# williamleif/GraphSAGE

Hardware: NVIDIA H100
Metric: seed_nodes_per_sec (higher is better)
Workload: dtype f32

## Files before the change

### graphsage_b200/_lib.py

```python
import ctypes
import os

import torch

_HERE = os.path.dirname(os.path.abspath(__file__))
LIB_PATH = os.path.join(_HERE, "csrc", "libgraphsage_b200.so")

ABI_VERSION = 2
GS_F32, GS_BF16, GS_F64 = 0, 1, 2
ACT_NONE, ACT_RELU = 0, 1
COMBINE_ADD, COMBINE_CONCAT = 0, 1
MATH_FP32_SIMT, MATH_TF32X3, MATH_TF32, MATH_BF16 = 0, 1, 2, 3
CSR_MEAN, CSR_MEAN_SELF, CSR_MAX = 0, 1, 2
MAX_SEGMENTS = 4

c_i32, c_i64, c_u64, c_vp = ctypes.c_int32, ctypes.c_int64, ctypes.c_uint64, ctypes.c_void_p


class Segment(ctypes.Structure):
    _fields_ = [("self_ids", c_vp), ("neigh_ids", c_vp), ("self_row0", c_i64), ("neigh_row0", c_i64),
                ("n", c_i64), ("k", c_i32), ("_pad", c_i32), ("out_row0", c_i64)]


MAX_SHARDS = 16


class ShardedTable(ctypes.Structure):
    _fields_ = [("base", c_vp * MAX_SHARDS), ("row_start", c_i64 * (MAX_SHARDS + 1)), ("n_shards", c_i32),
                ("my_shard", c_i32), ("n_global_rows", c_i64), ("zero_row", c_i64), ("remap", c_vp)]


class GemmPart(ctypes.Structure):
    _fields_ = [("A", c_vp), ("lda", c_i64), ("K", c_i32), ("B", c_vp), ("ldb", c_i64), ("N", c_i32)]


MAX_EMBED_LISTS = 8
MAX_UNIQUE_SAMPLED = 1024
UNIQUE_DRAW_BUDGET = 1 << 20
WALK_MAX_WALKS = 1 << 20
WALK_MAX_LEN = 33


class EmbedGradList(ctypes.Structure):
    _fields_ = [("ids", c_vp), ("grad", c_vp), ("ldg", c_i64), ("n", c_i64), ("group", c_i32), ("scale", ctypes.c_float)]


class DropoutSite(ctypes.Structure):
    _fields_ = [("seed", c_u64), ("call", ctypes.c_uint32), ("rate", ctypes.c_float), ("call_dev", c_vp)]
# ... 28 lines not shown
    "gs_ipc_import": (c_i32, [ctypes.c_char_p, ctypes.POINTER(c_vp)]),
    "gs_ipc_close": (c_i32, [c_vp]),
    "gs_gather_rows_f32": (c_i32, [c_vp, c_i32, c_i64, c_i32, c_i64, c_vp, c_i64, c_i64, c_vp, c_i64, c_vp]),
    "gs_cast_rows_bf16": (c_i32, [c_vp, c_i64, c_i32, c_i64, c_vp, c_i64, c_vp]),
    "gs_rmat_degrees": (c_i32, [c_i32, c_i64, ctypes.c_double, ctypes.c_double, ctypes.c_double, ctypes.c_double,
                                ctypes.c_double, c_u64, c_u64, c_u64, c_u64, c_vp, c_vp]),
    "gs_rmat_fill": (c_i32, [c_i32, c_i64, ctypes.c_double, ctypes.c_double, ctypes.c_double, ctypes.c_double, c_u64, c_u64,
                             c_u64, c_u64, c_vp, c_vp, c_vp, c_i64, c_i64, c_vp]),
    "gs_segment_max": (c_i32, [c_vp, c_i64, c_i32, c_i32, c_i64, c_vp, c_i64, c_vp]),
    "gs_sage_gemm_workspace_bytes": (c_i64, [c_i64, ctypes.POINTER(GemmPart), c_i32, c_i32]),
    "gs_sage_gemm": (c_i32, [c_i64, ctypes.POINTER(GemmPart), c_i32, c_i32, c_vp, c_i32, c_i32, c_vp, c_i64, c_vp,
                             c_vp]),
    "gs_sage_gemm_pack": (c_i32, [ctypes.POINTER(GemmPart), c_i32, c_i32, c_vp, c_vp]),
    "gs_sage_gemm_prepacked": (c_i32, [c_i64, ctypes.POINTER(GemmPart), c_i32, c_i32, c_vp, c_i32, c_i32, c_vp, c_i64,
                                       c_vp, c_vp]),
    "gs_gather_mean_img_bytes": (c_i64, [c_i64, c_i32, c_i32]),
    "gs_gather_mean_img": (c_i32, [c_vp, c_i64, ctypes.POINTER(ShardedTable), c_i32, c_vp, c_i32, c_i64, ctypes.POINTER(Segment),
                                   c_i32, c_i32, c_i32, c_vp, c_vp]),
    "gs_sage_gemm_img": (c_i32, [c_i64, ctypes.POINTER(GemmPart), c_i32, c_i32, c_vp, c_i32, c_vp, c_i64, c_vp, c_vp, c_i32,
                                 c_vp]),
    "gs_sage_layer_small": (c_i32, [c_vp, c_i64, c_i32, c_i64, ctypes.POINTER(Segment), c_i32, ctypes.POINTER(GemmPart),
                                    c_i32, c_i32, c_vp, c_i32, c_i32, c_vp, c_i64, c_vp, c_u64, c_vp]),
    "gs_maxpool_mlp_workspace_bytes": (c_i64, [c_i32, c_i32]),
    "gs_maxpool_mlp_pack": (c_i32, [c_vp, c_i64, c_i32, c_i32, c_vp, c_vp]),
    "gs_maxpool_mlp_fused": (c_i32, [c_vp, c_i64, c_i32, c_i64, c_vp, c_i64, c_i64, c_i32, c_vp, c_vp, c_i32, c_vp, c_i64,
                                     c_vp]),
    "gs_meanpool_mlp_fused": (c_i32, [c_vp, c_i64, c_i32, c_i64, c_vp, c_i64, c_i64, c_i32, c_vp, c_vp, c_i32, c_vp, c_i64,
                                      c_vp]),
    "gs_pool_mlp_dp_bytes": (c_i64, [c_i64, c_i32, c_i32]),
    "gs_pool_mlp_backward_dp": (c_i32, [c_vp, c_i64, c_i32, c_i64, c_vp, c_i64, c_i64, c_i32, c_vp, c_vp, c_i32, c_vp, c_i64,
# ... 94 lines not shown
```

### graphsage_b200/aggregators.py

```python
import torch

from . import ops
from .inits import glorot, zeros
from .layers import Dense, Layer, act_code, identity, relu

_DEFAULT_MATH = [ops.MATH_FP32_SIMT]
_MATH_NAMES = {"fp32": ops.MATH_FP32_SIMT, "simt": ops.MATH_FP32_SIMT, "tf32x3": ops.MATH_TF32X3,
               "tf32": ops.MATH_TF32, "bf16": ops.MATH_BF16}


def set_default_math(mode):
    _DEFAULT_MATH[0] = _MATH_NAMES[mode] if isinstance(mode, str) else int(mode)


def _dropout(x, p):
    return torch.nn.functional.dropout(x, p=float(p), training=True) if p else x


def _dense_segment(n, k):
    return [ops.make_segment(n, k)]


def _rows(src, ids, row0, n, f32=False, out=None):
    if f32:
# ... 104 lines not shown
                             (means, self.neigh_input_dim, self.vars["neigh_weights"])], self._combine())

    def aggregate_rows(self, src, segments, final=None, src_persistent=False):
        if self.dropout:
            raise NotImplementedError("dropout > 0 uses the dense call path")
        y = self._small_layer(src, segments, [(None, self.input_dim, self.vars["self_weights"]),
                                              (None, self.neigh_input_dim, self.vars["neigh_weights"])],
                              self._combine(), False, final)
        if y is not None:
            return y
        y = self._image_layer(src, segments, [(None, self.input_dim, self.vars["self_weights"]),
                                              (None, self.neigh_input_dim, self.vars["neigh_weights"])],
                              self._combine(), False, True)
        if y is not None:
            return y
        xs, xm = ops.gather_mean(src, segments, want_self=True)
        return self._finish([(xs, self.input_dim, self.vars["self_weights"]),
                             (xm, self.neigh_input_dim, self.vars["neigh_weights"])], self._combine())


class GCNAggregator(_SageAggregator):

    def __init__(self, input_dim, output_dim, neigh_input_dim=None, dropout=0., bias=False, act=relu, name=None,
                 concat=False, device="cuda", **kwargs):
        super(GCNAggregator, self).__init__(**kwargs)
        self.dropout = dropout
        self.bias = bias
        self.act = act
        self.concat = concat
        if neigh_input_dim is None:
            neigh_input_dim = input_dim
# ... 222 lines not shown
```

### graphsage_b200/csrc/common.cuh

```cuda
#pragma once
#include <cuda_runtime.h>
#include <math.h>
#include <stdint.h>
#include <stdio.h>
#include <string.h>

#include "../../include/graphsage_b200.h"

namespace gs {

void set_error(const char* fmt, ...);
int32_t cuda_fail(cudaError_t e, const char* what);
int32_t tuning(const char* key, int32_t dflt);
int32_t ensure_dyn_smem(const void* kernel, int bytes);

#define GS_REQUIRE(cond, ...)            \
  do {                                   \
    if (!(cond)) {                       \
      gs::set_error(__VA_ARGS__);        \
      return GS_ERR_INVALID_ARG;         \
    }                                    \
  } while (0)

#define GS_CUDA(expr)                                        \
// ... 143 lines not shown
__device__ __forceinline__ void bulk_wait_read() {
  asm volatile("cp.async.bulk.wait_group.read %0;" ::"n"(N) : "memory");
}
template <int N>
__device__ __forceinline__ void bulk_wait() {
  asm volatile("cp.async.bulk.wait_group %0;" ::"n"(N) : "memory");
}

__device__ __forceinline__ float4 ldg_nc_f4(const float4* p) {
  float4 r;
  asm volatile("ld.global.nc.L1::no_allocate.v4.f32 {%0,%1,%2,%3}, [%4];"
               : "=f"(r.x), "=f"(r.y), "=f"(r.z), "=f"(r.w)
               : "l"(p));
  return r;
}
#endif

}
```

### graphsage_b200/csrc/gather.cu

```cuda
#include "common.cuh"

namespace gs {

struct SegTable {
  gs_segment s[GS_MAX_SEGMENTS];
  int32_t n_segments;
  int64_t total_rows;
};

__device__ __forceinline__ int find_segment(const SegTable& t, int64_t r, int64_t& local) {
  int si = 0;
  int64_t base = 0, end = 0;
#pragma unroll
  for (int q = 0; q < GS_MAX_SEGMENTS - 1; ++q) {
    if (q < t.n_segments - 1) {
      end += t.s[q].n;
      if (r >= end) {
        base = end;
        si = q + 1;
      }
    }
  }
  local = r - base;
  return si;
// ... 221 lines not shown
  const int kb = c >> 3, chunk = c & 7;
  const int64_t mt = orow >> 7;
  const int r = (int)(orow & 127);
  unsigned char* dst = im.base + ((((int64_t)part * im.n_mtiles + mt) * im.kblocks + kb) * 2) * 16384 +
                       (uint32_t)(r * 128 + ((chunk ^ (r & 7)) << 4));
  uint4 hi, lo;
  hi.x = __float_as_uint(v.x) & 0xFFFFE000u; hi.y = __float_as_uint(v.y) & 0xFFFFE000u;
  hi.z = __float_as_uint(v.z) & 0xFFFFE000u; hi.w = __float_as_uint(v.w) & 0xFFFFE000u;
  lo.x = __float_as_uint(v.x - __uint_as_float(hi.x)) & 0xFFFFE000u; lo.y = __float_as_uint(v.y - __uint_as_float(hi.y)) & 0xFFFFE000u;
  lo.z = __float_as_uint(v.z - __uint_as_float(hi.z)) & 0xFFFFE000u; lo.w = __float_as_uint(v.w - __uint_as_float(hi.w)) & 0xFFFFE000u;
  *reinterpret_cast<uint4*>(dst) = hi;
  *reinterpret_cast<uint4*>(dst + 16384) = lo;
}

template <class Rows, bool kDrop>
__global__ void __launch_bounds__(192) gather_mean_tma2_kernel(const __grid_constant__ Rows rows_of, int F,
                                                               const __grid_constant__ SegTable tab,
                                                               int include_self, float* __restrict__ out_self,
                                                               float* __restrict__ out_mean, int64_t out_pitch,
                                                               int row_bytes, const __grid_constant__ GatherImg img,
                                                               const __grid_constant__ DropTab drop) {
  extern __shared__ __align__(128) unsigned char smem[];
  __shared__ __align__(8) uint64_t bar[2];
  __shared__ uint32_t drop_off[2 * GS_MAX_SEGMENTS];
  if (threadIdx.x == 0) {
    mbar_init(&bar[0], 1);
    mbar_init(&bar[1], 1);
    fence_mbar_init();
  }
  if constexpr (kDrop) {
    if (threadIdx.x < 2 * GS_MAX_SEGMENTS) {
      const int s = threadIdx.x % GS_MAX_SEGMENTS;
      drop_off[threadIdx.x] = drop_call_offset(threadIdx.x < GS_MAX_SEGMENTS ? drop.neigh[s] : drop.self[s]);
    }
  }
  __syncthreads();
  const int ncol4 = (int)(out_pitch >> 2);
  const int row_f4 = row_bytes >> 4;
  const size_t buf_bytes = (size_t)kGroupRows * row_bytes;

  int64_t r_issue = blockIdx.x;
  int g_issue = 0;
  auto issue = [&](int buf) -> bool {
    if (r_issue >= tab.total_rows) return false;
    int64_t i;
    const gs_segment& sg = tab.s[find_segment(tab, r_issue, i)];
    const int k = sg.k;
    const int rows_total = k + 1;
    const int first = g_issue * kGroupRows;
    const int cnt = min(kGroupRows, rows_total - first);
    if (threadIdx.x < 32) {
      if (threadIdx.x == 0) mbar_expect_tx(&bar[buf], (uint32_t)(cnt * row_bytes));
      __syncwarp();
      for (int j = threadIdx.x; j < cnt; j += 32) {
        const int jj = first + j;
        int64_t id;
        if (jj < k) id = sg.neigh_ids ? (int64_t)sg.neigh_ids[i * k + jj] : sg.neigh_row0 + i * k + jj;
        else id = sg.self_ids ? (int64_t)sg.self_ids[i] : sg.self_row0 + i;
        bulk_g2s(smem + buf * buf_bytes + (size_t)j * row_bytes, rows_of.row(id), (uint32_t)row_bytes, &bar[buf]);
      }
    }
    if (first + cnt >= rows_total) { r_issue += gridDim.x; g_issue = 0; } else { ++g_issue; }
    return true;
  };

  uint32_t phase[2] = {0u, 0u};
  int buf = 0;
  bool have = issue(0);
  int64_t r = blockIdx.x;
  int g = 0;
  float4 acc[2];
  acc[0] = acc[1] = make_float4(0.f, 0.f, 0.f, 0.f);
  while (have) {
    const bool have_next = issue(buf ^ 1);
    int64_t i;
    const int si = find_segment(tab, r, i);
    const gs_segment& sg = tab.s[si];
    const int k = sg.k;
    const int rows_total = k + 1;
    const int first = g * kGroupRows;
    const int cnt = min(kGroupRows, rows_total - first);
    const bool last = first + cnt >= rows_total;
    mbar_wait(&bar[buf], phase[buf]);
    phase[buf] ^= 1u;
    const float4* rows = reinterpret_cast<const float4*>(smem + buf * buf_bytes);
    const int nn = last ? cnt - 1 : cnt;
    DropSite nsite{};
    if constexpr (kDrop) nsite = with_call_offset(drop.neigh[si], drop_off[si]);
#pragma unroll
    for (int q = 0; q < 2; ++q) {
      const int c = threadIdx.x + q * blockDim.x;
      if (c < ncol4 && c * 4 < F) {
        float4 a = acc[q];
        for (int j = 0; j < nn; ++j) {
          float4 v = rows[j * row_f4 + c];
          if constexpr (kDrop) v = drop4(nsite, i * k + first + j, (uint32_t)c, v);
          a.x += v.x; a.y += v.y; a.z += v.z; a.w += v.w;
        }
        acc[q] = a;
      }
    }
    if (last) {
      const int64_t orow = sg.out_row0 + i;
      const int ncol_img = img.base ? img.kblocks * 8 : 0;
#pragma unroll
      for (int q = 0; q < 2; ++q) {
        const int c = threadIdx.x + q * blockDim.x;
        if (c < ncol4 || c < ncol_img) {
          float4 a = make_float4(0.f, 0.f, 0.f, 0.f), sv = a;
          if (c < ncol4 && c * 4 < F) {
            a = acc[q];
            sv = rows[(cnt - 1) * row_f4 + c];
            if constexpr (kDrop) sv = drop4(with_call_offset(drop.self[si], drop_off[GS_MAX_SEGMENTS + si]), i, (uint32_t)c, sv);
            const float div = (float)(k + (include_self ? 1 : 0));
            if (include_self) { a.x += sv.x; a.y += sv.y; a.z += sv.z; a.w += sv.w; }
            a.x /= div; a.y /= div; a.z /= div; a.w /= div;
            a = mask_tail(a, c * 4, F);
            sv = mask_tail(sv, c * 4, F);
          }
          if (c < ncol4) {
            if (out_mean) reinterpret_cast<float4*>(out_mean + orow * out_pitch)[c] = a;
            if (out_self) reinterpret_cast<float4*>(out_self + orow * out_pitch)[c] = sv;
          }
          if (c < ncol_img) {
            if (img.want_self) gather_img_store(img, 0, orow, c, sv);
            gather_img_store(img, img.want_self ? 1 : 0, orow, c, a);
          }
          if (c < ncol4) acc[q] = make_float4(0.f, 0.f, 0.f, 0.f);
// ... 1011 lines not shown
```

### graphsage_b200/csrc/gemm_api.cu

```cuda
#include "common.cuh"

namespace gs {
int32_t sage_gemm_simt(int64_t M, const gs_gemm_part* parts, int32_t n_parts, int32_t combine, const float* bias,
                       int32_t act, float* out, int64_t ldo, cudaStream_t st);
int64_t sage_gemm_tc_workspace(int64_t M, const gs_gemm_part* parts, int32_t n_parts, int32_t math);
int32_t sage_gemm_tc_img(int64_t M, const gs_gemm_part* parts, int32_t n_parts, int32_t combine, const float* bias, int32_t act,
                         float* out, int64_t ldo, const void* workspace, const void* a_images, int32_t a_part0, cudaStream_t st);
int32_t sage_gemm_tc(int64_t M, const gs_gemm_part* parts, int32_t n_parts, int32_t combine, const float* bias,
                     int32_t act, int32_t math, float* out, int64_t ldo, const void* workspace, cudaStream_t st);
int32_t sage_gemm_tc_pack(const gs_gemm_part* parts, int32_t n_parts, int32_t math, void* workspace, cudaStream_t st);
}

static int32_t check_parts(int64_t M, const gs_gemm_part* parts, int32_t n_parts, int32_t combine, bool need_a = true) {
  GS_REQUIRE(M >= 0, "gs_sage_gemm: M < 0");
  GS_REQUIRE(parts && (n_parts == 1 || n_parts == 2), "gs_sage_gemm: n_parts must be 1 or 2 (got %d)", n_parts);
  GS_REQUIRE(combine == GS_COMBINE_ADD || combine == GS_COMBINE_CONCAT, "gs_sage_gemm: combine=%d", combine);
  for (int i = 0; i < n_parts; ++i) {
    GS_REQUIRE(parts[i].K >= 1 && parts[i].N >= 1, "gs_sage_gemm: part %d has K=%d N=%d", i, parts[i].K, parts[i].N);
    GS_REQUIRE(parts[i].lda >= parts[i].K && parts[i].ldb >= parts[i].N, "gs_sage_gemm: part %d leading dims too small", i);
    GS_REQUIRE(M == 0 || ((parts[i].A || !need_a) && parts[i].B), "gs_sage_gemm: part %d NULL operand", i);
  }
  if (n_parts == 2 && combine == GS_COMBINE_ADD)
    GS_REQUIRE(parts[0].N == parts[1].N, "gs_sage_gemm: ADD needs equal N (%d vs %d)", parts[0].N, parts[1].N);
  return GS_OK;
// ... 5 lines not shown
  if (!parts_host || n_parts < 1 || n_parts > 2 || M < 0) return -1;
  if (math == GS_MATH_FP32_SIMT) return 0;
  return gs::sage_gemm_tc_workspace(M, parts_host, n_parts, math);
}

static bool is_tc(int32_t math) { return math == GS_MATH_TF32X3 || math == GS_MATH_TF32 || math == GS_MATH_BF16; }

int32_t gs_sage_gemm_pack(const gs_gemm_part* parts_host, int32_t n_parts, int32_t math, void* workspace, void* stream) {
  int32_t rc = check_parts(1, parts_host, n_parts, GS_COMBINE_CONCAT, false);
  if (rc != GS_OK) return rc;
  if (math == GS_MATH_FP32_SIMT) return GS_OK;
  GS_REQUIRE(is_tc(math), "gs_sage_gemm_pack: unknown math mode %d", math);
  return gs::sage_gemm_tc_pack(parts_host, n_parts, math, workspace, (cudaStream_t)stream);
}

int32_t gs_sage_gemm_prepacked(int64_t M, const gs_gemm_part* parts_host, int32_t n_parts, int32_t combine,
                               const float* bias, int32_t act, int32_t math, float* out, int64_t ldo,
                               const void* workspace, void* stream) {
  int32_t rc = check_parts(M, parts_host, n_parts, combine);
  if (rc != GS_OK) return rc;
  if (M == 0) return GS_OK;
  GS_REQUIRE(out, "gs_sage_gemm: out is NULL");
  int ntot = parts_host[0].N + ((n_parts == 2 && combine == GS_COMBINE_CONCAT) ? parts_host[1].N : 0);
  GS_REQUIRE(ldo >= ntot, "gs_sage_gemm: ldo=%lld < output width %d", (long long)ldo, ntot);
  GS_REQUIRE(act == GS_ACT_NONE || act == GS_ACT_RELU, "gs_sage_gemm: act=%d", act);
  if (math == GS_MATH_FP32_SIMT)
    return gs::sage_gemm_simt(M, parts_host, n_parts, combine, bias, act, out, ldo, (cudaStream_t)stream);
  GS_REQUIRE(is_tc(math), "gs_sage_gemm: unknown math mode %d", math);
  return gs::sage_gemm_tc(M, parts_host, n_parts, combine, bias, act, math, out, ldo, workspace, (cudaStream_t)stream);
}

int32_t gs_sage_gemm_img(int64_t M, const gs_gemm_part* parts_host, int32_t n_parts, int32_t combine, const float* bias,
                         int32_t act, float* out, int64_t ldo, const void* workspace, const void* a_images,
                         int32_t a_part0, void* stream) {
  GS_REQUIRE(parts_host && n_parts >= 1 && n_parts <= 2, "gs_sage_gemm_img: n_parts must be 1 or 2");
  for (int i = 0; i < n_parts; ++i)
    GS_REQUIRE(parts_host[i].B && parts_host[i].K >= 1 && parts_host[i].N >= 1 && parts_host[i].ldb >= parts_host[i].N,
               "gs_sage_gemm_img: bad part %d", i);
  GS_REQUIRE(combine == GS_COMBINE_CONCAT || n_parts == 1 || parts_host[0].N == parts_host[1].N,
             "gs_sage_gemm_img: ADD needs equal output widths");
  if (M == 0) return GS_OK;
  GS_REQUIRE(M > 0 && out, "gs_sage_gemm_img: bad M / out");
  int ntot = parts_host[0].N + ((n_parts == 2 && combine == GS_COMBINE_CONCAT) ? parts_host[1].N : 0);
  GS_REQUIRE(ldo >= ntot, "gs_sage_gemm_img: ldo=%lld < output width %d", (long long)ldo, ntot);
// ... 17 lines not shown
```

### graphsage_b200/csrc/gemm_simt.cu

```cuda
#include "common.cuh"

namespace gs {

struct GemmParts {
  gs_gemm_part p[2];
  int32_t n_parts;
  int32_t combine;
};

constexpr int BM = 64, BN = 64, BK = 16;

__global__ void __launch_bounds__(256) sage_gemm_simt_kernel(int64_t M, const __grid_constant__ GemmParts gp,
                                                             const float* __restrict__ bias, int act,
                                                             float* __restrict__ out, int64_t ldo, int tiles_n0) {
  __shared__ float As[BK][BM + 4];
  __shared__ float Bs[BK][BN];
  const int tx = threadIdx.x & 15, ty = threadIdx.x >> 4;
  const int64_t m0 = (int64_t)blockIdx.x * BM;
  int part_lo = 0, part_hi = gp.n_parts;
  int n0, col_off = 0;
  if (gp.combine == GS_COMBINE_CONCAT && gp.n_parts == 2) {
    if ((int)blockIdx.y < tiles_n0) { part_hi = 1; n0 = blockIdx.y * BN; }
    else { part_lo = 1; n0 = ((int)blockIdx.y - tiles_n0) * BN; col_off = gp.p[0].N; }
  } else {
    n0 = blockIdx.y * BN;
  }
  const int N = gp.p[part_lo].N;
  float acc[4][4];
#pragma unroll
  for (int i = 0; i < 4; ++i)
#pragma unroll
    for (int j = 0; j < 4; ++j) acc[i][j] = 0.f;

  for (int pi = part_lo; pi < part_hi; ++pi) {
    const gs_gemm_part& P = gp.p[pi];
    for (int k0 = 0; k0 < P.K; k0 += BK) {
#pragma unroll
      for (int e = 0; e < 4; ++e) {
        int idx = threadIdx.x + e * 256;
        int r = idx >> 4, kk = idx & 15;
        int64_t gm = m0 + r;
        int gk = k0 + kk;
        As[kk][r] = (gm < M && gk < P.K) ? P.A[gm * P.lda + gk] : 0.f;
      }
#pragma unroll
      for (int e = 0; e < 4; ++e) {
        int idx = threadIdx.x + e * 256;
        int kk = idx >> 6, c = idx & 63;
        int gk = k0 + kk, gn = n0 + c;
        Bs[kk][c] = (gk < P.K && gn < N) ? P.B[(int64_t)gk * P.ldb + gn] : 0.f;
      }
      __syncthreads();
#pragma unroll
      for (int kk = 0; kk < BK; ++kk) {
        float a[4], b[4];
#pragma unroll
        for (int i = 0; i < 4; ++i) a[i] = As[kk][ty * 4 + i];
#pragma unroll
// ... 10 lines not shown
  for (int i = 0; i < 4; ++i) {
    int64_t gm = m0 + ty * 4 + i;
    if (gm >= M) continue;
#pragma unroll
    for (int j = 0; j < 4; ++j) {
      int gn = n0 + tx * 4 + j;
      if (gn >= N) continue;
      float v = acc[i][j];
      if (bias) v += bias[col_off + gn];
      if (act == GS_ACT_RELU) v = fmaxf(v, 0.f);
      out[gm * ldo + col_off + gn] = v;
    }
  }
}

int32_t sage_gemm_simt(int64_t M, const gs_gemm_part* parts, int32_t n_parts, int32_t combine, const float* bias,
                       int32_t act, float* out, int64_t ldo, cudaStream_t st) {
  GemmParts gp;
  memset(&gp, 0, sizeof(gp));
  gp.n_parts = n_parts;
  gp.combine = combine;
  for (int i = 0; i < n_parts; ++i) gp.p[i] = parts[i];
  int tiles_n0 = (parts[0].N + BN - 1) / BN;
  int tiles_n = tiles_n0;
  if (combine == GS_COMBINE_CONCAT && n_parts == 2) tiles_n += (parts[1].N + BN - 1) / BN;
  dim3 grid((unsigned)((M + BM - 1) / BM), (unsigned)tiles_n);
  sage_gemm_simt_kernel<<<grid, 256, 0, st>>>(M, gp, bias, act, out, ldo, tiles_n0);
  return launch_check("sage_gemm_simt_kernel");
}

}
```

### graphsage_b200/csrc/gemm_tc.cu

```cuda
#include "tc_common.cuh"

namespace gs {

constexpr int TC_THREADS = 256;

struct TcPart {
  const float* A;
  int64_t lda;
  int32_t K;
  int32_t N;
  int32_t kblocks;
  int32_t ntiles;
  int64_t img_off;
  const float* B;
  int64_t ldb;
};

struct TcParams {
  TcPart p[2];
  int32_t n_parts;
  int32_t combine;
  int64_t M;
  const float* bias;
  int32_t act;
  float* out;
  int64_t ldo;
  int32_t tiles_n0;
  const unsigned char* a_img;
  int32_t a_mtiles;
  int32_t a_part0;
};

template <int MODE>
__global__ void __launch_bounds__(256) pack_b_kernel(TcParams prm, unsigned char* __restrict__ ws) {
  constexpr int BK = MODE == 2 ? 64 : 32;
  constexpr int EPC = MODE == 2 ? 8 : 4;
  constexpr int NIMG = MODE == 0 ? 2 : 1;
  int unit = blockIdx.x;
  int pi = 0;
  if (prm.n_parts == 2 && unit >= prm.p[0].ntiles * prm.p[0].kblocks) {
    unit -= prm.p[0].ntiles * prm.p[0].kblocks;
    pi = 1;
  }
  const TcPart& P = prm.p[pi];
  const int nt = unit / P.kblocks, kb = unit % P.kblocks;
// ... 25 lines not shown
  }
}

template <int MODE>
struct TcCfg {
  static constexpr int BK = MODE == 2 ? 64 : 32;
  static constexpr int NIMG = MODE == 0 ? 2 : 1;
  static constexpr int IMG_BYTES = NIMG * TC_TILE_BYTES;
  static constexpr int STAGES = MODE == 0 ? 3 : 4;
  static constexpr int STAGE_BYTES = 2 * IMG_BYTES;
  static constexpr int SMEM_BYTES = STAGES * STAGE_BYTES + 1024;
  static constexpr int CPT = 4;
};

template <int MODE>
__device__ __forceinline__ void load_a_chunk(const TcPart& P, int64_t M, int64_t grow, int gcol, bool vec, float (&v)[8]) {
  constexpr int EPC = MODE == 2 ? 8 : 4;
#pragma unroll
  for (int e = 0; e < 8; ++e) v[e] = 0.f;
  if (grow >= M) return;
  const float* src = P.A + grow * P.lda + gcol;
  if (vec && gcol + EPC <= P.K) {
    float4 a = ldg_nc_f4(reinterpret_cast<const float4*>(src));
    v[0] = a.x; v[1] = a.y; v[2] = a.z; v[3] = a.w;
    if constexpr (EPC == 8) {
      float4 b = ldg_nc_f4(reinterpret_cast<const float4*>(src) + 1);
      v[4] = b.x; v[5] = b.y; v[6] = b.z; v[7] = b.w;
    }
  } else {
#pragma unroll
    for (int e = 0; e < EPC; ++e)
      if (gcol + e < P.K) v[e] = __ldg(src + e);
  }
}

template <int MODE>
// ... 49 lines not shown
  __syncthreads();

  auto post = [&](int it) {
    if (tid != 0 || it >= total_it) return;
    int pi, kb;
    locate(it, pi, kb);
    const TcPart& P = prm.p[pi];
    const int s = it % C::STAGES;
    unsigned char* st = smem + (size_t)s * C::STAGE_BYTES;
    mbar_expect_tx(&full[s], kImg ? 2 * C::IMG_BYTES : C::IMG_BYTES);
    bulk_g2s(st + C::IMG_BYTES, ws + P.img_off + ((int64_t)ntile * P.kblocks + kb) * C::IMG_BYTES, C::IMG_BYTES, &full[s]);
    if constexpr (kImg)
      bulk_g2s(st, prm.a_img + (((int64_t)(prm.a_part0 + pi) * prm.a_mtiles + blockIdx.x) * P.kblocks + kb) * C::IMG_BYTES,
               C::IMG_BYTES, &full[s]);
  };
  float cur[C::CPT][8];
  auto fetch = [&](int it) {
    int pi, kb;
    locate(it, pi, kb);
    const TcPart& P = prm.p[pi];
    const bool vec = ((P.lda & 3) == 0) && ((reinterpret_cast<uintptr_t>(P.A) & 15u) == 0);
#pragma unroll
    for (int i = 0; i < C::CPT; ++i) {
      const int q = tid + TC_THREADS * i;
      load_a_chunk<MODE>(P, prm.M, m0 + (q >> 3), kb * C::BK + (q & 7) * (MODE == 2 ? 8 : 4), vec, cur[i]);
    }
  };

  for (int j = 0; j < C::STAGES - 1; ++j) post(j);
  if constexpr (!kImg) fetch(0);

  float acc[64];
#pragma unroll
  for (int i = 0; i < 64; ++i) acc[i] = 0.f;
  for (int it = 0; it < total_it; ++it) {
    const int s = it % C::STAGES;
    unsigned char* st = smem + (size_t)s * C::STAGE_BYTES;
    if constexpr (!kImg) {
#pragma unroll
      for (int i = 0; i < C::CPT; ++i) {
// ... 119 lines not shown
  GS_REQUIRE(workspace != nullptr && (reinterpret_cast<uintptr_t>(workspace) & 127u) == 0,
             "gs_sage_gemm_img: packed weights missing or not 128-byte aligned");
  GS_REQUIRE(a_images != nullptr && (reinterpret_cast<uintptr_t>(a_images) & 1023u) == 0,
             "gs_sage_gemm_img: A images missing or not 1024-byte aligned");
  TcParams prm;
  fill_parts(prm, M, parts, n_parts, 0);
  for (int i = 1; i < n_parts; ++i)
    GS_REQUIRE(prm.p[i].K == prm.p[0].K, "gs_sage_gemm_img: every part must have the K of the gathered rows");
  prm.combine = combine; prm.bias = bias; prm.act = act; prm.out = out; prm.ldo = ldo;
  prm.a_img = (const unsigned char*)a_images;
  prm.a_mtiles = (int32_t)((M + TC_BM - 1) / TC_BM);
  prm.a_part0 = a_part0;
  return launch_tc<0, true>(prm, (const unsigned char*)workspace, st);
}

int32_t sage_gemm_tc(int64_t M, const gs_gemm_part* parts, int32_t n_parts, int32_t combine, const float* bias,
                     int32_t act, int32_t math, float* out, int64_t ldo, const void* workspace, cudaStream_t st) {
  GS_REQUIRE(workspace != nullptr, "gs_sage_gemm: tensor-core math modes need the workspace (gs_sage_gemm_workspace_bytes)");
  GS_REQUIRE((reinterpret_cast<uintptr_t>(workspace) & 127u) == 0, "gs_sage_gemm: workspace must be 128-byte aligned");
  const int mode = mode_of(math);
  TcParams prm;
  fill_parts(prm, M, parts, n_parts, mode);
  prm.combine = combine;
  prm.bias = bias;
  prm.act = act;
  prm.out = out;
  prm.ldo = ldo;
  const unsigned char* ws = (const unsigned char*)workspace;
  if (mode == 0) return launch_tc<0, false>(prm, ws, st);
  if (mode == 1) return launch_tc<1, false>(prm, ws, st);
  return launch_tc<2, false>(prm, ws, st);
}

}
```

### graphsage_b200/ops.py

```python
import torch

from . import _lib
from ._lib import (ACT_NONE, ACT_RELU, COMBINE_ADD, COMBINE_CONCAT, MATH_FP32_SIMT, MATH_TF32X3, MATH_TF32,
                   MATH_BF16, GemmPart, Segment, check, lib, ptr, require_cuda, stream_ptr)

_U64 = 2**64 - 1

PROBE = None
LAUNCHES = 0
STAGE_HOOK = None

CACHE_EPOCH = [0]
REPACK_ALWAYS = [False]


def _probe(name):
    if STAGE_HOOK is not None:
        STAGE_HOOK(name, "pre")
    if PROBE is None:
        return _PostHook(name) if STAGE_HOOK is not None else None
    e0, e1 = torch.cuda.Event(enable_timing=True), torch.cuda.Event(enable_timing=True)
    PROBE.setdefault(name, []).append((e0, e1))
    e0.record()
    return e1
# ... 416 lines not shown
    n_nodes = indptr.numel() - 1
    if rows is not None:
        rows = _i32(rows.reshape(-1), "rows")
    n, F = (n_nodes + 1 if rows is None else rows.numel()), src.shape[1]
    if out is None:
        out = torch.empty((n, pad_cols(F)), dtype=torch.float32, device=src.device)
    if out.dtype != torch.float32 or out.dim() != 2 or out.stride(1) != 1 or out.shape[0] < n:
        raise ValueError("out must be a row-major float32 [>= %d, .] CUDA matrix" % n)
    ev = _probe("csr_aggregate/%d" % n)
    check(lib().gs_csr_aggregate(ptr(src), _dtype_code(src), src.shape[0], F, src.stride(0), ptr(indptr), ptr(indices),
                                 n_nodes, ptr(rows), n, CSR_OPS[op], ptr(out), out.stride(0), stream_ptr()))
    _launched(1 if n else 0, ev)
    return out[:n, :F]


def _gemm_parts(parts):
    M = parts[0][0].shape[0] if parts[0][0] is not None else 0
    arr = (GemmPart * len(parts))()
    keep = []
    for i, (A, K, B) in enumerate(parts):
        require_cuda(A, B)
        if (A is not None and A.dtype != torch.float32) or B.dtype != torch.float32:
            raise TypeError("sage_gemm operands must be float32")
        if A is not None and (A.stride(1) != 1 or A.shape[0] != M or A.shape[1] < K):
            raise ValueError("bad A operand for part %d" % i)
        B = B.contiguous()
        if B.shape[0] != K:
            raise ValueError("part %d: B has %d rows, expected K=%d" % (i, B.shape[0], K))
        keep.append(B)
        arr[i] = GemmPart(ptr(A), A.stride(0) if A is not None else K, K, ptr(B), B.stride(0), B.shape[1])
    return M, arr, keep


class PackedWeights(object):

    def __init__(self):
        self.key, self.ws = None, None

    def get(self, parts, arr, math, dev):
# ... 7 lines not shown

    @staticmethod
    def _pack(parts, arr, math, dev, ws):
        nbytes = lib().gs_sage_gemm_workspace_bytes(1, arr, len(parts), math)
        if nbytes < 0:
            check(-1)
        if ws is None or ws.numel() < nbytes:
            ws = torch.empty((max(nbytes, 1),), dtype=torch.uint8, device=dev)
        check(lib().gs_sage_gemm_pack(arr, len(parts), math, ptr(ws), stream_ptr()))
        _launched(1)
        return ws


def sage_gemm(parts, combine=COMBINE_ADD, bias=None, act=ACT_NONE, math=MATH_FP32_SIMT, out=None, packed=None):
    M, arr, keep = _gemm_parts(parts)
    ntot = sum(p[2].shape[1] for p in parts) if (combine == COMBINE_CONCAT) else parts[0][2].shape[1]
    dev = parts[0][0].device
    if out is None:
        out = torch.empty((M, ntot), dtype=torch.float32, device=dev)
    if math == MATH_FP32_SIMT or packed is None:
        ws_bytes = lib().gs_sage_gemm_workspace_bytes(M, arr, len(parts), math)
        if ws_bytes < 0:
            check(-1)
        ws = torch.empty((ws_bytes,), dtype=torch.uint8, device=dev) if ws_bytes > 0 else None
        ev = _probe("sage_gemm/%d" % M)
        check(lib().gs_sage_gemm(M, arr, len(parts), combine, ptr(bias), act, math, ptr(out), out.stride(0), ptr(ws),
                                 stream_ptr()))
        _launched((2 if ws is not None else 1) if M else 0, ev)
        return out
    ws = packed.get(parts, arr, math, dev)
    ev = _probe("sage_gemm/%d" % M)
    check(lib().gs_sage_gemm_prepacked(M, arr, len(parts), combine, ptr(bias), act, math, ptr(out), out.stride(0),
                                       ptr(ws), stream_ptr()))
    _launched(1 if M else 0, ev)
    return out


SMALL_LAYER_MAX_ROWS = 2048


def sage_layer_small(src, seg, parts, combine=COMBINE_ADD, include_self=False, bias=None, act=ACT_NONE,
                     l2_normalize=False, counter_dev=None, counter_inc=0):
    require_cuda(src, bias, counter_dev)
    if src.dtype != torch.float32 or src.stride(1) != 1:
        raise ValueError("src must be row-major float32")
    _, arr, keep = _gemm_parts([(None, K, B) for (_, K, B) in parts])
    ntot = sum(p[2].shape[1] for p in parts) if (combine == COMBINE_CONCAT) else parts[0][2].shape[1]
    rows = seg.out_row0 + seg.n
# ... 365 lines not shown
```

### include/graphsage_b200.h

```cpp
#ifndef GRAPHSAGE_B200_H_
#define GRAPHSAGE_B200_H_

#include <stdint.h>

#ifdef __cplusplus
extern "C" {
#endif

#define GS_ABI_VERSION 2

typedef enum {
  GS_OK = 0,
  GS_ERR_INVALID_ARG = -1,
  GS_ERR_CUDA = -2,
  GS_ERR_UNSUPPORTED = -3
} gs_status;

typedef enum { GS_F32 = 0, GS_BF16 = 1, GS_F64 = 2 } gs_dtype;
typedef enum { GS_ACT_NONE = 0, GS_ACT_RELU = 1 } gs_act;
typedef enum {
  GS_COMBINE_ADD = 0,
  GS_COMBINE_CONCAT = 1
} gs_combine;
typedef enum {
// ... 110 lines not shown
  const float* B; int64_t ldb; int32_t N;
} gs_gemm_part;

int64_t gs_sage_gemm_workspace_bytes(int64_t M, const gs_gemm_part* parts_host, int32_t n_parts,
                                     int32_t math);
int32_t gs_sage_gemm(int64_t M, const gs_gemm_part* parts_host, int32_t n_parts, int32_t combine,
                     const float* bias, int32_t act, int32_t math, float* out, int64_t ldo,
                     void* workspace, void* stream);

int32_t gs_sage_gemm_pack(const gs_gemm_part* parts_host, int32_t n_parts, int32_t math, void* workspace,
                          void* stream);
int32_t gs_sage_gemm_prepacked(int64_t M, const gs_gemm_part* parts_host, int32_t n_parts, int32_t combine,
                               const float* bias, int32_t act, int32_t math, float* out, int64_t ldo,
                               const void* workspace, void* stream);

int64_t gs_gather_mean_img_bytes(int64_t rows, int32_t F, int32_t want_self);
int32_t gs_gather_mean_img(const void* src, int64_t n_src_rows, const gs_sharded_table* table_host, int32_t ids_are_locators,
                           const void* staging, int32_t F, int64_t pitch, const gs_segment* segments_host,
                           int32_t n_segments, int32_t include_self, int32_t want_self, void* images, void* stream);
int32_t gs_sage_gemm_img(int64_t M, const gs_gemm_part* parts_host, int32_t n_parts, int32_t combine, const float* bias,
                         int32_t act, float* out, int64_t ldo, const void* workspace, const void* a_images,
                         int32_t a_part0, void* stream);

int32_t gs_sage_layer_small(const float* src, int64_t n_src_rows, int32_t F, int64_t pitch,
                            const gs_segment* segment_host, int32_t include_self,
                            const gs_gemm_part* parts_host, int32_t n_parts, int32_t combine,
                            const float* bias, int32_t act, int32_t l2_normalize,
                            float* out, int64_t ldo, uint64_t* counter_dev, uint64_t counter_inc,
                            void* stream);

// ... 115 lines not shown
```

Before: 3.588 million.

## Read self rows by id inside the GEMM instead of gathering them

In the fallback aggregate path, self rows are no longer copied into a dense gathered matrix. The GEMM A-operand loader resolves each output row to a table row through per-segment id ranges. The gather-mean kernel skips loading the self row when it is not needed and gets a minBlocks launch bound. This removes a gather write and re-read of the self features, at the cost of indirect, less coalesced A loads and extra per-row index lookups in the GEMM. The sage_gemm path also now calls pack followed by the new rows entry.

```diff
diff --git a/graphsage_b200/_lib.py b/graphsage_b200/_lib.py
--- a/graphsage_b200/_lib.py
+++ b/graphsage_b200/_lib.py
@@ -32,6 +32,14 @@
 
 class GemmPart(ctypes.Structure):
     _fields_ = [("A", c_vp), ("lda", c_i64), ("K", c_i32), ("B", c_vp), ("ldb", c_i64), ("N", c_i32)]
+
+
+class RowRange(ctypes.Structure):
+    _fields_ = [("ids", c_vp), ("row0", c_i64), ("n", c_i64)]
+
+
+class GemmRowIds(ctypes.Structure):
+    _fields_ = [("n_table_rows", c_i64), ("n_ranges", c_i32), ("_pad", c_i32), ("ranges", RowRange * MAX_SEGMENTS)]
 
 
 MAX_EMBED_LISTS = 8
@@ -90,6 +98,8 @@
     "gs_sage_gemm_pack": (c_i32, [ctypes.POINTER(GemmPart), c_i32, c_i32, c_vp, c_vp]),
     "gs_sage_gemm_prepacked": (c_i32, [c_i64, ctypes.POINTER(GemmPart), c_i32, c_i32, c_vp, c_i32, c_i32, c_vp, c_i64,
                                        c_vp, c_vp]),
+    "gs_sage_gemm_rows": (c_i32, [c_i64, ctypes.POINTER(GemmPart), ctypes.POINTER(GemmRowIds), c_i32, c_i32, c_vp, c_i32, c_i32,
+                                  c_vp, c_i64, c_vp, c_vp]),
     "gs_gather_mean_img_bytes": (c_i64, [c_i64, c_i32, c_i32]),
     "gs_gather_mean_img": (c_i32, [c_vp, c_i64, ctypes.POINTER(ShardedTable), c_i32, c_vp, c_i32, c_i64, ctypes.POINTER(Segment),
                                    c_i32, c_i32, c_i32, c_vp, c_vp]),
diff --git a/graphsage_b200/aggregators.py b/graphsage_b200/aggregators.py
--- a/graphsage_b200/aggregators.py
+++ b/graphsage_b200/aggregators.py
@@ -142,7 +142,11 @@
                               self._combine(), False, True)
         if y is not None:
             return y
-        xs, xm = ops.gather_mean(src, segments, want_self=True)
+        if torch.is_tensor(src) and src.is_cuda and src.dtype == torch.float32 and all(s.self_ids is not None for s in segments):
+            _, xm = ops.gather_mean(src, segments, want_self=False)
+            xs = ops.TableRows(src, [(s.self_ids[:s.n], s.out_row0) for s in segments], xm.shape[0])
+        else:
+            xs, xm = ops.gather_mean(src, segments, want_self=True)
         return self._finish([(xs, self.input_dim, self.vars["self_weights"]),
                              (xm, self.neigh_input_dim, self.vars["neigh_weights"])], self._combine())
 
diff --git a/graphsage_b200/csrc/common.cuh b/graphsage_b200/csrc/common.cuh
--- a/graphsage_b200/csrc/common.cuh
+++ b/graphsage_b200/csrc/common.cuh
@@ -181,6 +181,20 @@
                : "l"(p));
   return r;
 }
+
+__device__ __forceinline__ int64_t gemm_a_row(const gs_gemm_row_ids& R, int64_t M, int64_t r) {
+  if (r >= M) return -1;
+  if (R.n_ranges == 0) return r;
+#pragma unroll
+  for (int s = 0; s < GS_MAX_SEGMENTS; ++s) {
+    const gs_row_range& g = R.ranges[s];
+    if (s < R.n_ranges && r >= g.row0 && r - g.row0 < g.n) {
+      const int64_t id = g.ids[r - g.row0];
+      return (id < 0 || id >= R.n_table_rows) ? R.n_table_rows - 1 : id;
+    }
+  }
+  return -1;
+}
 #endif
 
 }
diff --git a/graphsage_b200/csrc/gather.cu b/graphsage_b200/csrc/gather.cu
--- a/graphsage_b200/csrc/gather.cu
+++ b/graphsage_b200/csrc/gather.cu
@@ -259,7 +259,7 @@
 }
 
 template <class Rows, bool kDrop>
-__global__ void __launch_bounds__(192) gather_mean_tma2_kernel(const __grid_constant__ Rows rows_of, int F,
+__global__ void __launch_bounds__(192, 3) gather_mean_tma2_kernel(const __grid_constant__ Rows rows_of, int F,
                                                                const __grid_constant__ SegTable tab,
                                                                int include_self, float* __restrict__ out_self,
                                                                float* __restrict__ out_mean, int64_t out_pitch,
@@ -283,6 +283,7 @@
   const int ncol4 = (int)(out_pitch >> 2);
   const int row_f4 = row_bytes >> 4;
   const size_t buf_bytes = (size_t)kGroupRows * row_bytes;
+  const int self_rows = (include_self || out_self || (img.base && img.want_self)) ? 1 : 0;
 
   int64_t r_issue = blockIdx.x;
   int g_issue = 0;
@@ -291,7 +292,7 @@
     int64_t i;
     const gs_segment& sg = tab.s[find_segment(tab, r_issue, i)];
     const int k = sg.k;
-    const int rows_total = k + 1;
+    const int rows_total = k + self_rows;
     const int first = g_issue * kGroupRows;
     const int cnt = min(kGroupRows, rows_total - first);
     if (threadIdx.x < 32) {
@@ -322,14 +323,14 @@
     const int si = find_segment(tab, r, i);
     const gs_segment& sg = tab.s[si];
     const int k = sg.k;
-    const int rows_total = k + 1;
+    const int rows_total = k + self_rows;
     const int first = g * kGroupRows;
     const int cnt = min(kGroupRows, rows_total - first);
     const bool last = first + cnt >= rows_total;
     mbar_wait(&bar[buf], phase[buf]);
     phase[buf] ^= 1u;
     const float4* rows = reinterpret_cast<const float4*>(smem + buf * buf_bytes);
-    const int nn = last ? cnt - 1 : cnt;
+    const int nn = last ? cnt - self_rows : cnt;
     DropSite nsite{};
     if constexpr (kDrop) nsite = with_call_offset(drop.neigh[si], drop_off[si]);
 #pragma unroll
@@ -355,8 +356,10 @@
           float4 a = make_float4(0.f, 0.f, 0.f, 0.f), sv = a;
           if (c < ncol4 && c * 4 < F) {
             a = acc[q];
-            sv = rows[(cnt - 1) * row_f4 + c];
-            if constexpr (kDrop) sv = drop4(with_call_offset(drop.self[si], drop_off[GS_MAX_SEGMENTS + si]), i, (uint32_t)c, sv);
+            if (self_rows) {
+              sv = rows[(cnt - 1) * row_f4 + c];
+              if constexpr (kDrop) sv = drop4(with_call_offset(drop.self[si], drop_off[GS_MAX_SEGMENTS + si]), i, (uint32_t)c, sv);
+            }
             const float div = (float)(k + (include_self ? 1 : 0));
             if (include_self) { a.x += sv.x; a.y += sv.y; a.z += sv.z; a.w += sv.w; }
             a.x /= div; a.y /= div; a.z /= div; a.w /= div;
diff --git a/graphsage_b200/csrc/gemm_api.cu b/graphsage_b200/csrc/gemm_api.cu
--- a/graphsage_b200/csrc/gemm_api.cu
+++ b/graphsage_b200/csrc/gemm_api.cu
@@ -1,13 +1,14 @@
 #include "common.cuh"
 
 namespace gs {
-int32_t sage_gemm_simt(int64_t M, const gs_gemm_part* parts, int32_t n_parts, int32_t combine, const float* bias,
-                       int32_t act, float* out, int64_t ldo, cudaStream_t st);
+int32_t sage_gemm_simt(int64_t M, const gs_gemm_part* parts, const gs_gemm_row_ids* row_ids, int32_t n_parts,
+                       int32_t combine, const float* bias, int32_t act, float* out, int64_t ldo, cudaStream_t st);
 int64_t sage_gemm_tc_workspace(int64_t M, const gs_gemm_part* parts, int32_t n_parts, int32_t math);
 int32_t sage_gemm_tc_img(int64_t M, const gs_gemm_part* parts, int32_t n_parts, int32_t combine, const float* bias, int32_t act,
                          float* out, int64_t ldo, const void* workspace, const void* a_images, int32_t a_part0, cudaStream_t st);
-int32_t sage_gemm_tc(int64_t M, const gs_gemm_part* parts, int32_t n_parts, int32_t combine, const float* bias,
-                     int32_t act, int32_t math, float* out, int64_t ldo, const void* workspace, cudaStream_t st);
+int32_t sage_gemm_tc(int64_t M, const gs_gemm_part* parts, const gs_gemm_row_ids* row_ids, int32_t n_parts, int32_t combine,
+                     const float* bias, int32_t act, int32_t math, float* out, int64_t ldo, const void* workspace,
+                     cudaStream_t st);
 int32_t sage_gemm_tc_pack(const gs_gemm_part* parts, int32_t n_parts, int32_t math, void* workspace, cudaStream_t st);
 }
 
@@ -43,20 +44,40 @@
   return gs::sage_gemm_tc_pack(parts_host, n_parts, math, workspace, (cudaStream_t)stream);
 }
 
-int32_t gs_sage_gemm_prepacked(int64_t M, const gs_gemm_part* parts_host, int32_t n_parts, int32_t combine,
-                               const float* bias, int32_t act, int32_t math, float* out, int64_t ldo,
-                               const void* workspace, void* stream) {
+int32_t gs_sage_gemm_rows(int64_t M, const gs_gemm_part* parts_host, const gs_gemm_row_ids* row_ids_host, int32_t n_parts,
+                          int32_t combine, const float* bias, int32_t act, int32_t math, float* out, int64_t ldo,
+                          const void* workspace, void* stream) {
   int32_t rc = check_parts(M, parts_host, n_parts, combine);
   if (rc != GS_OK) return rc;
+  gs_gemm_row_ids rid[2];
+  memset(rid, 0, sizeof(rid));
+  for (int i = 0; row_ids_host && i < n_parts; ++i) {
+    const gs_gemm_row_ids& R = row_ids_host[i];
+    if (R.n_ranges == 0) continue;
+    GS_REQUIRE(R.n_ranges > 0 && R.n_ranges <= GS_MAX_SEGMENTS, "gs_sage_gemm_rows: part %d has n_ranges=%d (max %d)", i,
+               R.n_ranges, GS_MAX_SEGMENTS);
+    GS_REQUIRE(R.n_table_rows >= 1 && R.n_table_rows < ((int64_t)1 << 31), "gs_sage_gemm_rows: part %d n_table_rows=%lld", i,
+               (long long)R.n_table_rows);
+    for (int s = 0; s < R.n_ranges; ++s)
+      GS_REQUIRE(R.ranges[s].n >= 0 && R.ranges[s].row0 >= 0 && (R.ranges[s].ids || R.ranges[s].n == 0),
+                 "gs_sage_gemm_rows: part %d range %d is invalid", i, s);
+    rid[i] = R;
+  }
   if (M == 0) return GS_OK;
   GS_REQUIRE(out, "gs_sage_gemm: out is NULL");
   int ntot = parts_host[0].N + ((n_parts == 2 && combine == GS_COMBINE_CONCAT) ? parts_host[1].N : 0);
   GS_REQUIRE(ldo >= ntot, "gs_sage_gemm: ldo=%lld < output width %d", (long long)ldo, ntot);
   GS_REQUIRE(act == GS_ACT_NONE || act == GS_ACT_RELU, "gs_sage_gemm: act=%d", act);
   if (math == GS_MATH_FP32_SIMT)
-    return gs::sage_gemm_simt(M, parts_host, n_parts, combine, bias, act, out, ldo, (cudaStream_t)stream);
+    return gs::sage_gemm_simt(M, parts_host, rid, n_parts, combine, bias, act, out, ldo, (cudaStream_t)stream);
   GS_REQUIRE(is_tc(math), "gs_sage_gemm: unknown math mode %d", math);
-  return gs::sage_gemm_tc(M, parts_host, n_parts, combine, bias, act, math, out, ldo, workspace, (cudaStream_t)stream);
+  return gs::sage_gemm_tc(M, parts_host, rid, n_parts, combine, bias, act, math, out, ldo, workspace, (cudaStream_t)stream);
+}
+
+int32_t gs_sage_gemm_prepacked(int64_t M, const gs_gemm_part* parts_host, int32_t n_parts, int32_t combine,
+                               const float* bias, int32_t act, int32_t math, float* out, int64_t ldo,
+                               const void* workspace, void* stream) {
+  return gs_sage_gemm_rows(M, parts_host, nullptr, n_parts, combine, bias, act, math, out, ldo, workspace, stream);
 }
 
 int32_t gs_sage_gemm_img(int64_t M, const gs_gemm_part* parts_host, int32_t n_parts, int32_t combine, const float* bias,
diff --git a/graphsage_b200/csrc/gemm_simt.cu b/graphsage_b200/csrc/gemm_simt.cu
--- a/graphsage_b200/csrc/gemm_simt.cu
+++ b/graphsage_b200/csrc/gemm_simt.cu
@@ -6,6 +6,7 @@
   gs_gemm_part p[2];
   int32_t n_parts;
   int32_t combine;
+  gs_gemm_row_ids rid[2];
 };
 
 constexpr int BM = 64, BN = 64, BK = 16;
@@ -34,14 +35,16 @@
 
   for (int pi = part_lo; pi < part_hi; ++pi) {
     const gs_gemm_part& P = gp.p[pi];
+    int64_t arow[4];
+#pragma unroll
+    for (int e = 0; e < 4; ++e) arow[e] = gemm_a_row(gp.rid[pi], M, m0 + ((threadIdx.x + e * 256) >> 4));
     for (int k0 = 0; k0 < P.K; k0 += BK) {
 #pragma unroll
       for (int e = 0; e < 4; ++e) {
         int idx = threadIdx.x + e * 256;
         int r = idx >> 4, kk = idx & 15;
-        int64_t gm = m0 + r;
         int gk = k0 + kk;
-        As[kk][r] = (gm < M && gk < P.K) ? P.A[gm * P.lda + gk] : 0.f;
+        As[kk][r] = (arow[e] >= 0 && gk < P.K) ? P.A[arow[e] * P.lda + gk] : 0.f;
       }
 #pragma unroll
       for (int e = 0; e < 4; ++e) {
@@ -82,13 +85,14 @@
   }
 }
 
-int32_t sage_gemm_simt(int64_t M, const gs_gemm_part* parts, int32_t n_parts, int32_t combine, const float* bias,
-                       int32_t act, float* out, int64_t ldo, cudaStream_t st) {
+int32_t sage_gemm_simt(int64_t M, const gs_gemm_part* parts, const gs_gemm_row_ids* row_ids, int32_t n_parts,
+                       int32_t combine, const float* bias, int32_t act, float* out, int64_t ldo, cudaStream_t st) {
   GemmParts gp;
   memset(&gp, 0, sizeof(gp));
   gp.n_parts = n_parts;
   gp.combine = combine;
   for (int i = 0; i < n_parts; ++i) gp.p[i] = parts[i];
+  for (int i = 0; row_ids && i < n_parts; ++i) gp.rid[i] = row_ids[i];
   int tiles_n0 = (parts[0].N + BN - 1) / BN;
   int tiles_n = tiles_n0;
   if (combine == GS_COMBINE_CONCAT && n_parts == 2) tiles_n += (parts[1].N + BN - 1) / BN;
diff --git a/graphsage_b200/csrc/gemm_tc.cu b/graphsage_b200/csrc/gemm_tc.cu
--- a/graphsage_b200/csrc/gemm_tc.cu
+++ b/graphsage_b200/csrc/gemm_tc.cu
@@ -29,6 +29,7 @@
   const unsigned char* a_img;
   int32_t a_mtiles;
   int32_t a_part0;
+  gs_gemm_row_ids rid[2];
 };
 
 template <int MODE>
@@ -84,12 +85,12 @@
 };
 
 template <int MODE>
-__device__ __forceinline__ void load_a_chunk(const TcPart& P, int64_t M, int64_t grow, int gcol, bool vec, float (&v)[8]) {
+__device__ __forceinline__ void load_a_chunk(const TcPart& P, int64_t arow, int gcol, bool vec, float (&v)[8]) {
   constexpr int EPC = MODE == 2 ? 8 : 4;
 #pragma unroll
   for (int e = 0; e < 8; ++e) v[e] = 0.f;
-  if (grow >= M) return;
-  const float* src = P.A + grow * P.lda + gcol;
+  if (arow < 0) return;
+  const float* src = P.A + arow * P.lda + gcol;
   if (vec && gcol + EPC <= P.K) {
     float4 a = ldg_nc_f4(reinterpret_cast<const float4*>(src));
     v[0] = a.x; v[1] = a.y; v[2] = a.z; v[3] = a.w;
@@ -169,6 +170,15 @@
       bulk_g2s(st, prm.a_img + (((int64_t)(prm.a_part0 + pi) * prm.a_mtiles + blockIdx.x) * P.kblocks + kb) * C::IMG_BYTES,
                C::IMG_BYTES, &full[s]);
   };
+  int64_t arow_lo[C::CPT], arow_hi[C::CPT];
+  if constexpr (!kImg) {
+#pragma unroll
+    for (int i = 0; i < C::CPT; ++i) {
+      const int64_t r = m0 + ((tid + TC_THREADS * i) >> 3);
+      arow_lo[i] = gemm_a_row(prm.rid[part_lo], prm.M, r);
+      arow_hi[i] = part_hi - part_lo == 2 ? gemm_a_row(prm.rid[part_lo + 1], prm.M, r) : -1;
+    }
+  }
   float cur[C::CPT][8];
   auto fetch = [&](int it) {
     int pi, kb;
@@ -178,7 +188,7 @@
 #pragma unroll
     for (int i = 0; i < C::CPT; ++i) {
       const int q = tid + TC_THREADS * i;
-      load_a_chunk<MODE>(P, prm.M, m0 + (q >> 3), kb * C::BK + (q & 7) * (MODE == 2 ? 8 : 4), vec, cur[i]);
+      load_a_chunk<MODE>(P, pi == part_lo ? arow_lo[i] : arow_hi[i], kb * C::BK + (q & 7) * (MODE == 2 ? 8 : 4), vec, cur[i]);
     }
   };
 
@@ -328,13 +338,15 @@
   return launch_tc<0, true>(prm, (const unsigned char*)workspace, st);
 }
 
-int32_t sage_gemm_tc(int64_t M, const gs_gemm_part* parts, int32_t n_parts, int32_t combine, const float* bias,
-                     int32_t act, int32_t math, float* out, int64_t ldo, const void* workspace, cudaStream_t st) {
+int32_t sage_gemm_tc(int64_t M, const gs_gemm_part* parts, const gs_gemm_row_ids* row_ids, int32_t n_parts, int32_t combine,
+                     const float* bias, int32_t act, int32_t math, float* out, int64_t ldo, const void* workspace,
+                     cudaStream_t st) {
   GS_REQUIRE(workspace != nullptr, "gs_sage_gemm: tensor-core math modes need the workspace (gs_sage_gemm_workspace_bytes)");
   GS_REQUIRE((reinterpret_cast<uintptr_t>(workspace) & 127u) == 0, "gs_sage_gemm: workspace must be 128-byte aligned");
   const int mode = mode_of(math);
   TcParams prm;
   fill_parts(prm, M, parts, n_parts, mode);
+  for (int i = 0; row_ids && i < n_parts; ++i) prm.rid[i] = row_ids[i];
   prm.combine = combine;
   prm.bias = bias;
   prm.act = act;
diff --git a/graphsage_b200/ops.py b/graphsage_b200/ops.py
--- a/graphsage_b200/ops.py
+++ b/graphsage_b200/ops.py
@@ -2,7 +2,7 @@
 
 from . import _lib
 from ._lib import (ACT_NONE, ACT_RELU, COMBINE_ADD, COMBINE_CONCAT, MATH_FP32_SIMT, MATH_TF32X3, MATH_TF32,
-                   MATH_BF16, GemmPart, Segment, check, lib, ptr, require_cuda, stream_ptr)
+                   MATH_BF16, GemmPart, GemmRowIds, RowRange, Segment, check, lib, ptr, require_cuda, stream_ptr)
 
 _U64 = 2**64 - 1
 
@@ -454,15 +454,45 @@
     return out[:n, :F]
 
 
+class TableRows(object):
+    __slots__ = ("table", "ranges", "M")
+
+    def __init__(self, table, ranges, M):
+        require_cuda(table)
+        if table.dtype != torch.float32 or table.dim() != 2 or table.stride(1) != 1:
+            raise ValueError("the row table must be a row-major float32 matrix")
+        if len(ranges) > _lib.MAX_SEGMENTS:
+            raise ValueError("at most %d id ranges" % _lib.MAX_SEGMENTS)
+        self.table, self.M = table, int(M)
+        self.ranges = [(_i32(ids.reshape(-1), "ids"), int(row0)) for ids, row0 in ranges]
+        require_cuda(*[ids for ids, _ in self.ranges])
+
+    @property
+    def device(self):
+        return self.table.device
+
+    def c_struct(self):
+        r = GemmRowIds(self.table.shape[0], len(self.ranges), 0)
+        for s, (ids, row0) in enumerate(self.ranges):
+            r.ranges[s] = RowRange(ptr(ids), row0, ids.numel())
+        return r
+
+
 def _gemm_parts(parts):
-    M = parts[0][0].shape[0] if parts[0][0] is not None else 0
+    A0 = parts[0][0]
+    M = A0.M if isinstance(A0, TableRows) else (A0.shape[0] if A0 is not None else 0)
     arr = (GemmPart * len(parts))()
     keep = []
     for i, (A, K, B) in enumerate(parts):
+        by_id = isinstance(A, TableRows)
+        if by_id:
+            if A.M != M:
+                raise ValueError("bad A operand for part %d" % i)
+            A = A.table
         require_cuda(A, B)
         if (A is not None and A.dtype != torch.float32) or B.dtype != torch.float32:
             raise TypeError("sage_gemm operands must be float32")
-        if A is not None and (A.stride(1) != 1 or A.shape[0] != M or A.shape[1] < K):
+        if A is not None and (A.stride(1) != 1 or (A.shape[0] != M and not by_id) or A.shape[1] < K):
             raise ValueError("bad A operand for part %d" % i)
         B = B.contiguous()
         if B.shape[0] != K:
@@ -500,24 +530,38 @@
 
 def sage_gemm(parts, combine=COMBINE_ADD, bias=None, act=ACT_NONE, math=MATH_FP32_SIMT, out=None, packed=None):
     M, arr, keep = _gemm_parts(parts)
+    rid = None
+    if any(isinstance(p[0], TableRows) for p in parts):
+        rid = (GemmRowIds * len(parts))()
+        for i, p in enumerate(parts):
+            if isinstance(p[0], TableRows):
+                rid[i] = p[0].c_struct()
     ntot = sum(p[2].shape[1] for p in parts) if (combine == COMBINE_CONCAT) else parts[0][2].shape[1]
     dev = parts[0][0].device
     if out is None:
         out = torch.empty((M, ntot), dtype=torch.float32, device=dev)
+
+    def run(ws):
+        if rid is None:
+            return lib().gs_sage_gemm_prepacked(M, arr, len(parts), combine, ptr(bias), act, math, ptr(out), out.stride(0),
+                                                ptr(ws), stream_ptr())
+        return lib().gs_sage_gemm_rows(M, arr, rid, len(parts), combine, ptr(bias), act, math, ptr(out), out.stride(0),
+                                       ptr(ws), stream_ptr())
+
     if math == MATH_FP32_SIMT or packed is None:
         ws_bytes = lib().gs_sage_gemm_workspace_bytes(M, arr, len(parts), math)
         if ws_bytes < 0:
             check(-1)
         ws = torch.empty((ws_bytes,), dtype=torch.uint8, device=dev) if ws_bytes > 0 else None
         ev = _probe("sage_gemm/%d" % M)
-        check(lib().gs_sage_gemm(M, arr, len(parts), combine, ptr(bias), act, math, ptr(out), out.stride(0), ptr(ws),
-                                 stream_ptr()))
+        if M and ws is not None:
+            check(lib().gs_sage_gemm_pack(arr, len(parts), math, ptr(ws), stream_ptr()))
+        check(run(ws))
         _launched((2 if ws is not None else 1) if M else 0, ev)
         return out
     ws = packed.get(parts, arr, math, dev)
     ev = _probe("sage_gemm/%d" % M)
-    check(lib().gs_sage_gemm_prepacked(M, arr, len(parts), combine, ptr(bias), act, math, ptr(out), out.stride(0),
-                                       ptr(ws), stream_ptr()))
+    check(run(ws))
     _launched(1 if M else 0, ev)
     return out
 
diff --git a/include/graphsage_b200.h b/include/graphsage_b200.h
--- a/include/graphsage_b200.h
+++ b/include/graphsage_b200.h
@@ -148,6 +148,21 @@
                                const float* bias, int32_t act, int32_t math, float* out, int64_t ldo,
                                const void* workspace, void* stream);
 
+typedef struct {
+  const int32_t* ids;
+  int64_t row0;
+  int64_t n;
+} gs_row_range;
+typedef struct {
+  int64_t n_table_rows;
+  int32_t n_ranges;
+  int32_t _pad;
+  gs_row_range ranges[GS_MAX_SEGMENTS];
+} gs_gemm_row_ids;
+int32_t gs_sage_gemm_rows(int64_t M, const gs_gemm_part* parts_host, const gs_gemm_row_ids* row_ids_host, int32_t n_parts,
+                          int32_t combine, const float* bias, int32_t act, int32_t math, float* out, int64_t ldo,
+                          const void* workspace, void* stream);
+
 int64_t gs_gather_mean_img_bytes(int64_t rows, int32_t F, int32_t want_self);
 int32_t gs_gather_mean_img(const void* src, int64_t n_src_rows, const gs_sharded_table* table_host, int32_t ids_are_locators,
                            const void* staging, int32_t F, int64_t pitch, const gs_segment* segments_host,
```

Measured after the change: 3.756 million (median of 6 runs). +4.7%, better.
